# courtois-neuromod/phantom_vlb

Measured on AMD Instinct MI355X. Metric: clips/sec fine-tune VideoLLaMA2-7B+LoRA->2k-voxel head, 1/2/4/8 MI355X, higher is better.
Workload: dtype bf16; 1 GPU; configs[2]: VideoLLaMA2-7B + LoRA r=16 + 2k-voxel head, bf16; clips_per_gpu=3, global_batch=3, seq_len=2048, frames=12, num_target=2048, weights=random-init, comm=none

## Files before the change

### include/vlb.h

```cpp
#ifndef VLB_H
#define VLB_H

#include <stdint.h>

#ifdef __cplusplus
extern "C" {
#endif
#if defined(__GNUC__) || defined(__clang__)
#pragma GCC visibility push(default)
#endif

#define VLB_OK 0
#define VLB_ERR_INVALID (-1)
#define VLB_ERR_LAUNCH (-2)

#define VLB_ABI_VERSION 2

#define VLB_ACT_NONE 0
#define VLB_ACT_QUICK_GELU 1
#define VLB_ACT_GELU 2
#define VLB_ACT_SILU 3
#define VLB_ACT_SWIGLU_PAIR 4
#define VLB_ACT_SWIGLU_BWD 5

// ... 8 lines not shown
                     const void* bias, const void* residual, int ldr, int act, const void* A2, int lda2,
                     const void* W2, int ldw2, int K2, void* ws, int64_t ws_bytes, void* stream);
int vlb_gemm_swiglu_save(const void* A, int lda, const void* W_il, int ldw, void* H, int ldh, void* GU, int ldgu, int M, int N,
                         int K, const void* A2, int lda2, const void* W2_il, int ldw2, int K2, void* ws, int64_t ws_bytes,
                         void* stream);
int64_t vlb_gemm_workspace_bytes(void);
int vlb_gemm_plan(int M, int N, int K, int K2, int with_workspace);

int vlb_gemm_bf16_masked_pair(const void* A, int lda, const void* W, int ldw, void* C, int ldc, int M, int N, int K,
                              const void* A2, int lda2, const void* W2, int ldw2, float drop_p, uint32_t seed,
                              void* stream);

int vlb_gemm_bf16_masked_pair_ws(const void* A, int lda, const void* W, int ldw, void* C, int ldc, int M, int N, int K,
                                 const void* A2, int lda2, const void* W2, int ldw2, float drop_p, uint32_t seed,
                                 void* ws, int64_t ws_bytes, void* stream);

int vlb_gemm_masked_pair_swiglu_bwd(const void* dY, int lddy, const void* Wt, int ldw, const void* gu, int ldgu, void* dgu,
                                    int lddgu, int M, int ff, int K, const void* U, int ldu, const void* At, int ldat,
                                    float drop_p, uint32_t seed, void* ws, int64_t ws_bytes, void* stream);

int vlb_gemm_kernel_choice(int M, int N, int K, int K2);

int vlb_transpose_bf16(const void* in, void* out, int R, int C, void* stream);

int vlb_attention_fwd(const void* q, int ldq, const void* k, int ldk, const void* v, int ldv, void* out, int ldo,
                      float* lse, const uint8_t* key_mask, int B, int S, int Hq, int Hkv, int D, int causal,
                      float scale, const int* cu_rows, void* stream);

int vlb_attention_bwd(const void* q, int ldq, const void* k, int ldk, const void* v, int ldv, const void* out,
                      int ldo, const void* dout, int lddo, const float* lse, const uint8_t* key_mask, void* dq,
                      int lddq, void* dk, int lddk, void* dv, int lddv, float* delta, float* dq_acc, int B, int S,
                      int Hq, int Hkv, int D, int causal, float scale, const int* cu_rows, int total_rows,
                      void* stream);

int vlb_rmsnorm_fwd(const void* x, const void* w, void* y, int rows, int dim, float eps, void* stream);
int vlb_rmsnorm_bwd(const void* x, const void* w, const void* dy, const void* dx_in, void* dx, int rows, int dim,
                    float eps, void* stream);
int vlb_layernorm_fwd(const void* x, const void* w, const void* b, const void* residual, void* y, int rows, int dim,
                      float eps, int act, void* stream);

int vlb_rope_inplace(void* x, int ld, const float* cos_t, const float* sin_t, int rows, int S, int heads, int D,
                     int sign, const int* pos, void* stream);
int vlb_swiglu_fwd(const void* gu, void* out, int rows, int ff, void* stream);
int vlb_swiglu_bwd(const void* gu, const void* dout, void* dgu, int rows, int ff, void* stream);
int vlb_add_bf16(const void* a, const void* b, void* y, int64_t n, void* stream);

int vlb_patchify(const float* vision, void* patches, int N, int H, int W, int P, int Kpad, void* stream);
int vlb_vit_assemble(const void* patch_emb, const void* cls, const void* pos, void* tokens, int N, int G, int D,
                     void* stream);
int vlb_drop_cls(const void* tokens, void* out, int N, int G, int D, void* stream);

int vlb_dwconv3x3(const void* x, const void* w, void* y, int N, int H, int W, int C, void* stream);
int vlb_se_pool(const void* x, void* pooled, int N, int HW, int C, void* stream);
int vlb_se_scale(const void* x, const void* gate, void* y, int N, int HW, int C, void* stream);
int vlb_im2col3d_k2s2p1(const void* x, void* cols, int B, int T, int H, int W, int C, void* stream);

int vlb_splice_embed(const int64_t* ids, const void* embed_w, const void* video_tokens, void* embeds,
                     uint8_t* key_mask, int* err_flag, int B, int L, int Nv, int D, int64_t video_id, int vocab,
                     const int* cu_rows, int* row_pos, void* stream);
int vlb_weight_mask(const int64_t* padvals, const double* vis_w, const double* lang_w, float* wmask, int B, int F,
                    int Lw, int tokens_per_frame, int S, int round_bf16, void* stream);

int vlb_head_partial_rows(int S);
int64_t vlb_head_ws_floats(int B, int S, int E, int V);
int vlb_head_fwd(const void* hidden, const float* wmask, const void* ln1_w, const void* ln1_b, const void* ln2_w,
                 const void* ln2_b, const void* ridge_w, const void* ridge_b, const float* y, const float* keep_scale,
// ... 204 lines not shown
```

### phantom_vlb_amd/_lib.py

```python
from __future__ import annotations

import ctypes
import os
from ctypes import c_char_p, c_double, c_float, c_int, c_int64, c_void_p

import torch

_HERE = os.path.dirname(os.path.abspath(__file__))
LIB_PATH = os.environ.get("VLB_LIB") or os.path.join(_HERE, "libvlb.so")
IS_PRODUCT_LIB = os.path.abspath(LIB_PATH) == os.path.join(_HERE, "libvlb.so")

P, I, F, L, D = c_void_p, c_int, c_float, c_int64, c_double

SIGNATURES = {
    "vlb_abi_version": [],
    "vlb_last_error": [],
    "vlb_gemm_bf16": [P, I, P, I, P, I, I, I, I, P, P, I, I, P, I, P, I, I, P],
    "vlb_gemm_bf16_ws": [P, I, P, I, P, I, I, I, I, P, P, I, I, P, I, P, I, I, P, L, P],
    "vlb_gemm_swiglu_save": [P, I, P, I, P, I, P, I, I, I, I, P, I, P, I, I, P, L, P],
    "vlb_gemm_workspace_bytes": [],
    "vlb_gemm_plan": [I, I, I, I, I],
    "vlb_gemm_kernel_choice": [I, I, I, I],
    "vlb_transpose_bf16": [P, P, I, I, P],
    "vlb_attention_fwd": [P, I, P, I, P, I, P, I, P, P, I, I, I, I, I, I, F, P, P],
    "vlb_attention_bwd": [P, I, P, I, P, I, P, I, P, I, P, P, P, I, P, I, P, I, P, P, I, I, I, I, I, I, F, P, I, P],
    "vlb_rmsnorm_fwd": [P, P, P, I, I, F, P],
    "vlb_rmsnorm_bwd": [P, P, P, P, P, I, I, F, P],
    "vlb_layernorm_fwd": [P, P, P, P, P, I, I, F, I, P],
    "vlb_rope_inplace": [P, I, P, P, I, I, I, I, I, P, P],
    "vlb_swiglu_fwd": [P, P, I, I, P],
    "vlb_swiglu_bwd": [P, P, P, I, I, P],
    "vlb_add_bf16": [P, P, P, L, P],
    "vlb_patchify": [P, P, I, I, I, I, I, P],
    "vlb_vit_assemble": [P, P, P, P, I, I, I, P],
    "vlb_drop_cls": [P, P, I, I, I, P],
    "vlb_dwconv3x3": [P, P, P, I, I, I, I, P],
    "vlb_se_pool": [P, P, I, I, I, P],
    "vlb_se_scale": [P, P, P, I, I, I, P],
    "vlb_im2col3d_k2s2p1": [P, P, I, I, I, I, I, P],
    "vlb_splice_embed": [P, P, P, P, P, P, I, I, I, I, L, I, P, P, P],
    "vlb_weight_mask": [P, P, P, P, I, I, I, I, I, I, P],
    "vlb_head_partial_rows": [I],
    "vlb_head_ws_floats": [I, I, I, I],
    "vlb_head_fwd": [P] * 19 + [I, I, I, I, F, F, P, P],
    "vlb_head_bwd": [P] * 24 + [I, I, I, I, F, F, F, F, P, I, P],
    "vlb_feature_cache_store": [P] * 5 + [I, I, I, P],
    "vlb_head_fwd_cached": [P] * 19 + [I, I, I, I, F, F, P],
    "vlb_head_bwd_cached": [P] * 20 + [I, I, I, F, F, F, F, P],
    "vlb_head_loss_fwd": [P] * 6 + [I, I, I, I, I, F, P],
    "vlb_head_bwd_loss": [P] * 24 + [I, I, I, I, F, F, F, F, P, I, P, I, P],
    "vlb_head_bwd_cached_loss": [P] * 20 + [I, I, I, F, F, F, F, P, I, P],
    "vlb_head_grouped_ws_floats": [I, I, I, I],
    "vlb_head_fwd_grouped": [P] * 22 + [I, I, I, I, I, F, F, I, P],
    "vlb_head_bwd_grouped": [P] * 22 + [I, I, I, I, F, F, F, F, I, P],
    "vlb_head_pool": [P] * 6 + [I, I, I, F, P, P],
    "vlb_feature_cache_gather": [P] * 5 + [I, I, I, P],
    "vlb_head_mix_fwd": [P] * 4 + [I, I, I, P],
    "vlb_head_mix_ws_floats": [I, I, I],
# ... 118 lines not shown
```

### phantom_vlb_amd/backbone.py

```python
from __future__ import annotations

import math

import torch

from . import ops
from .geometry import Geometry, VIDEO_TOKEN_ID, decoder_linears

BF16 = torch.bfloat16
V_PRE = "model.vision_tower.vision_tower.vision_model"
M_PRE = "model.mm_projector"


def _bf(t, dev):
    return t.detach().to(device=dev, dtype=BF16).contiguous()


class Weights:

    def __init__(self, g: Geometry, sd: dict, device, keep_transposed: bool = False, gate_up_interleaved: bool | None = None):
        self.g = g
        self.dev = device
        d = device
        w = sd[f"{V_PRE}.embeddings.patch_embedding.weight"].reshape(g.vit_dim, -1)
        wp = torch.zeros(g.vit_dim, g.patch_k_padded, dtype=w.dtype, device=w.device)
        wp[:, :g.patch_k] = w
        self.patch_w = _bf(wp, d)
        self.cls = _bf(sd[f"{V_PRE}.embeddings.class_embedding"], d)
        self.pos = _bf(sd[f"{V_PRE}.embeddings.position_embedding.weight"], d)
        self.pre_ln = (_bf(sd[f"{V_PRE}.pre_layrnorm.weight"], d), _bf(sd[f"{V_PRE}.pre_layrnorm.bias"], d))
        self.vit = []
        for i in range(g.vit_layers_run):
            p = f"{V_PRE}.encoder.layers.{i}"
            a = f"{p}.self_attn"
            self.vit.append(dict(
                ln1=(_bf(sd[f"{p}.layer_norm1.weight"], d), _bf(sd[f"{p}.layer_norm1.bias"], d)),
                ln2=(_bf(sd[f"{p}.layer_norm2.weight"], d), _bf(sd[f"{p}.layer_norm2.bias"], d)),
                wqkv=_bf(torch.cat([sd[f"{a}.q_proj.weight"], sd[f"{a}.k_proj.weight"], sd[f"{a}.v_proj.weight"]], 0), d),
                bqkv=_bf(torch.cat([sd[f"{a}.q_proj.bias"], sd[f"{a}.k_proj.bias"], sd[f"{a}.v_proj.bias"]], 0), d),
                wo=_bf(sd[f"{a}.out_proj.weight"], d), bo=_bf(sd[f"{a}.out_proj.bias"], d),
                w1=_bf(sd[f"{p}.mlp.fc1.weight"], d), b1=_bf(sd[f"{p}.mlp.fc1.bias"], d),
                w2=_bf(sd[f"{p}.mlp.fc2.weight"], d), b2=_bf(sd[f"{p}.mlp.fc2.bias"], d)))
        def stage(prefix):
            blocks = []
# ... 158 lines not shown
        y = ops.layernorm(y, *blk["bn2"], g.proj_eps, act=ops.ACT_SILU)
        s = ops.se_pool(y, N, H * H, C)
        s = ops.gemm(s, blk["se1"], bias=blk["se1b"], act=ops.ACT_SILU)
        s = ops.gemm(s, blk["se2"], bias=blk["se2b"])
        y = ops.se_scale(y, s, N, H * H, C, out=y)
        y = ops.gemm(y, blk["conv3"])
        sc = x
        if "ds" in blk:
            sc = ops.layernorm(ops.gemm(x, blk["ds"]), *blk["dsbn"], g.proj_eps)
        return ops.layernorm(y, *blk["bn3"], g.proj_eps, residual=sc, act=ops.ACT_SILU)

    def connector(self, feats, B):
        g, w = self.g, self.w
        x = feats
        for blk in w.s1:
            x = self._bottleneck(x, blk, B * g.num_frames, g.grid)
        cols = ops.im2col3d(x, B, g.num_frames, g.grid, g.grid, g.dim)
        x = ops.gemm(cols, w.sampler_w, bias=w.sampler_b, act=ops.ACT_SILU)
        for blk in w.s2:
            x = self._bottleneck(x, blk, B * g.ds_frames, g.ds_grid)
        x = ops.gemm(x, w.ro0[0], bias=w.ro0[1], act=ops.ACT_GELU)
        return ops.gemm(x, w.ro2[0], bias=w.ro2[1])

    def attention(self, qkv, key_mask, B, layout=None, need_lse=False):
        g, w = self.g, self.w
        qd, kd = g.q_dim, g.kv_dim
        ops.rope_(qkv, w.rope_cos, w.rope_sin, B, g.max_len, g.heads + g.kv_heads, g.head_dim,
                  pos=None if layout is None else layout.pos)
        return ops.attention_fwd(qkv[:, :qd], qkv[:, qd:qd + kd], qkv[:, qd + kd:], B, g.max_len, g.heads, g.kv_heads,
                                 g.head_dim, True, g.head_dim ** -0.5, key_mask=key_mask, need_lse=need_lse, layout=layout)

    def attention_bwd(self, qkv, a, d_a, lse, key_mask, B, layout, delta):
        g, w = self.g, self.w
        dqkv = ops.attention_bwd(qkv, g.q_dim, g.kv_dim, a, d_a, lse, key_mask, B, g.max_len, g.heads, g.kv_heads,
                                 g.head_dim, True, g.head_dim ** -0.5, layout=layout, delta=delta)
        ops.rope_(dqkv, w.rope_cos, w.rope_sin, B, g.max_len, g.heads + g.kv_heads, g.head_dim, sign=-1,
                  pos=None if layout is None else layout.pos)
        return dqkv

    def decoder_layer(self, x, lw, key_mask, B, S, save=None, layout=None):
        g = self.g
        assert S == g.max_len, "the decoder runs at the geometry's sequence length (rope tables, attention)"
        h = ops.rmsnorm(x, lw["in_norm"], g.rms_eps)
        qkv = ops.gemm(h, lw["wqkv"])
        a = self.attention(qkv, key_mask, B, layout)
        x = ops.gemm(a, lw["wo"], residual=x)
        h = ops.rmsnorm(x, lw["post_norm"], g.rms_eps)
        if lw.get("wgu_il") is not None:
            h = ops.gemm(h, lw["wgu_il"], act=ops.ACT_SWIGLU_PAIR)
        else:
            h = ops.swiglu(ops.gemm(h, lw["wgu"]))
        return ops.gemm(h, lw["wdown"], residual=x)

    def named_modules(self):
        from .litmodule import _LinearInfo
        g = self.g
        for i in range(g.vit_layers):
            p = f"{V_PRE}.encoder.layers.{i}"
            for n in ("q_proj", "k_proj", "v_proj", "out_proj"):
                yield f"{p}.self_attn.{n}", _LinearInfo(g.vit_dim, g.vit_dim)
            yield f"{p}.mlp.fc1", _LinearInfo(g.vit_ff, g.vit_dim)
            yield f"{p}.mlp.fc2", _LinearInfo(g.vit_dim, g.vit_ff)
        for n in ("readout.0", "readout.2"):
            yield f"{M_PRE}.{n}", _LinearInfo(g.dim, g.dim)
        for i in range(g.layers):
            p = f"model.layers.{i}"
# ... 155 lines not shown
```

### phantom_vlb_amd/csrc/attention.hip

```cpp
#include "common.hpp"

namespace {

constexpr int KV = 64;
constexpr int QW = 32;
constexpr int NW = 4;
constexpr int QB = QW * NW;
constexpr float NEG = -1e30f;

typedef short s16x4 __attribute__((ext_vector_type(4)));

__device__ __forceinline__ s16x4 tr_read_asm(const char* lds_ptr) {
  s16x4 v;
  const unsigned a = (unsigned)(uintptr_t)(const char __attribute__((address_space(3)))*)lds_ptr;
  asm volatile("ds_read_b64_tr_b16 %0, %1" : "=v"(v) : "v"(a));
  return v;
}
__device__ __forceinline__ void lds_wait_all() {
  asm volatile("s_waitcnt lgkmcnt(0)" ::: "memory");
  __builtin_amdgcn_sched_barrier(0);
}
__device__ __forceinline__ bf16x8 join8(s16x4 lo, s16x4 hi) {
  typedef short s16x8 __attribute__((ext_vector_type(8)));
  return __builtin_bit_cast(bf16x8, (s16x8)__builtin_shufflevector(lo, hi, 0, 1, 2, 3, 4, 5, 6, 7));
// ... 421 lines not shown
        for (int dt = 0; dt < 4; ++dt)
          dvt[dt] = __builtin_amdgcn_mfma_f32_32x32x16_bf16(join8(ra[dt][0], ra[dt][1]), pb[s], dvt[dt], 0, 0, 0);
#pragma unroll
        for (int dt = 0; dt < 4; ++dt)
#pragma unroll
          for (int e = 0; e < 2; ++e) ra[dt][e] = tr_read_asm(qt + qt_rd[dt][e] + 16 * s * ROWB);
        lds_wait_all();
#pragma unroll
        for (int dt = 0; dt < 4; ++dt)
          dkt[dt] = __builtin_amdgcn_mfma_f32_32x32x16_bf16(join8(ra[dt][0], ra[dt][1]), dsb[s], dkt[dt], 0, 0, 0);
      }
    }
    asm volatile("s_waitcnt vmcnt(0)" ::: "memory");
    asm volatile("s_waitcnt lgkmcnt(0)" ::: "memory");
    __builtin_amdgcn_s_barrier();
  }

  if (key < Sb) {
    bf16* dkp = gsz == 1 ? p.dk + (row0 + key) * p.lddk + hkv * D : part + ((row0 + key) * p.Hq + hq) * (2 * D);
    bf16* dvp = gsz == 1 ? p.dv + (row0 + key) * p.lddv + hkv * D : dkp + D;
#pragma unroll
    for (int dt = 0; dt < 4; ++dt)
#pragma unroll
      for (int g = 0; g < 4; ++g) {
        bf16x4 a, c;
#pragma unroll
        for (int e = 0; e < 4; ++e) { a[e] = (bf16)dkt[dt][4 * g + e]; c[e] = (bf16)dvt[dt][4 * g + e]; }
        *reinterpret_cast<bf16x4*>(dkp + 32 * dt + 8 * g + 4 * h) = a;
        *reinterpret_cast<bf16x4*>(dvp + 32 * dt + 8 * g + 4 * h) = c;
      }
  }
}

__global__ __launch_bounds__(256) void attn_dkdv_reduce_kernel(const bf16* __restrict__ part, bf16* __restrict__ dk, int lddk,
                                                               bf16* __restrict__ dv, int lddv, int Hq, int Hkv, int64_t total) {
  const int64_t i = blockIdx.x * (int64_t)blockDim.x + threadIdx.x;
  if (i >= total) return;
  const int c = i & 15, which = (i >> 4) & 1;
  const int hkv = (int)((i >> 5) % Hkv);
  const int64_t row = (i >> 5) / Hkv;
  const int gsz = Hq / Hkv;
  float acc[8] = {0.f, 0.f, 0.f, 0.f, 0.f, 0.f, 0.f, 0.f};
  const bf16* src = part + (row * Hq + (int64_t)hkv * gsz) * 256 + which * 128 + c * 8;
  for (int j = 0; j < gsz; ++j) {
    const bf16x8 v = *reinterpret_cast<const bf16x8*>(src + (int64_t)j * 256);
#pragma unroll
    for (int e = 0; e < 8; ++e) acc[e] += (float)v[e];
  }
  bf16x8 o;
#pragma unroll
  for (int e = 0; e < 8; ++e) o[e] = (bf16)acc[e];
  bf16* dst = which ? dv + row * lddv : dk + row * lddk;
  *reinterpret_cast<bf16x8*>(dst + hkv * 128 + c * 8) = o;
}

struct AttnDqArgs {
  const bf16* q; const bf16* k; const bf16* v; const bf16* dout;
  const float* lse; const float* delta; const uint8_t* mask; const int* cu;
  bf16* dq;
  int ldq, ldk, ldv, lddo, lddq;
  int B, S, Hq, Hkv;
  float scale;
};

template <bool CAUSAL>
__global__ __launch_bounds__(256, 2) void attn_bwd_dq_kernel(AttnDqArgs p) {
  constexpr int D = 128, ROWB = 256, TILE = KV * ROWB, KS = 8, DT = 4;
  extern __shared__ __attribute__((aligned(16))) char smem[];

  const int tid = threadIdx.x, lane = tid & 63;
  const int wave = __builtin_amdgcn_readfirstlane(tid >> 6);
  const int nqb = (p.S + QB - 1) / QB;
  const int per_qb = p.Hq * p.B, slot = blockIdx.x / per_qb;
  const int qb = CAUSAL ? (nqb - 1 - slot) : slot;
  const int hq = xcd_head((blockIdx.x % per_qb) % p.Hq, p.Hq), b = (blockIdx.x % per_qb) / p.Hq;
  const int hkv = hq / (p.Hq / p.Hkv);
  const int Sb = p.cu ? p.cu[b + 1] - p.cu[b] : p.S;
  const int64_t row0 = p.cu ? p.cu[b] : (int64_t)b * p.S;
  if (qb * QB >= Sb) return;
  const int q0 = qb * QB + wave * QW;
  const int ql = lane & 31, h = lane >> 5;
  const int qrow = q0 + ql;
  const int qr = min(qrow, Sb - 1);

  bf16x8 qf[KS], dof[KS];
  {
    const bf16* qp = p.q + (row0 + qr) * p.ldq + hq * D + 8 * h;
    const bf16* dp = p.dout + (row0 + qr) * p.lddo + hq * D + 8 * h;
#pragma unroll
    for (int ks = 0; ks < KS; ++ks) {
      qf[ks] = *reinterpret_cast<const bf16x8*>(qp + 16 * ks);
      dof[ks] = *reinterpret_cast<const bf16x8*>(dp + 16 * ks);
    }
  }
  const float lse_q = p.lse[((int64_t)b * p.Hq + hq) * p.S + qr];
  const float delta_q = p.delta[((int64_t)b * p.Hq + hq) * p.S + qr];
  const float c2 = p.scale * 1.44269504088896341f;
  const float lse2 = (lse_q > -1e37f) ? lse_q * 1.44269504088896341f : 1e37f;

  f32x16 dqt[DT];
#pragma unroll
  for (int i = 0; i < DT; ++i)
#pragma unroll
    for (int r = 0; r < 16; ++r) dqt[i][r] = 0.f;

  const int q_hi = min(qb * QB + QB, Sb) - 1;
  const int ntiles = CAUSAL ? (q_hi / KV + 1) : (Sb + KV - 1) / KV;
  const bf16* kbase = p.k + row0 * p.ldk + hkv * D;
  const bf16* vbase = p.v + row0 * p.ldv + hkv * D;

  const int sr = lane >> 4, sp = lane & 15;
  auto stage = [&](int buf, int t) {
    char* kb = smem + buf * 2 * TILE; char* vb = kb + TILE;
#pragma unroll
    for (int i = 0; i < 4; ++i) {
      const int r = (4 * i + wave) * 4 + sr;
      const int key = min(t * KV + r, Sb - 1);
      glds16(kbase + (int64_t)key * p.ldk + (sp ^ sw2(r)) * 8, kb + (4 * i + wave) * 1024);
      glds16(vbase + (int64_t)key * p.ldv + (sp ^ sw2(r)) * 8, vb + (4 * i + wave) * 1024);
    }
  };
  stage(0, 0);
  asm volatile("s_waitcnt vmcnt(0)" ::: "memory");
  __syncthreads();

  const int g1 = (lane >> 4) & 1, li = lane & 15, tq = li >> 2, tp = li & 3;
  int row_rd[KS];
#pragma unroll
  for (int ks = 0; ks < KS; ++ks) row_rd[ks] = ql * ROWB + (((2 * ks + h) ^ sw2(ql)) << 4);
  int tr_rd[DT][2];
#pragma unroll
  for (int dt = 0; dt < DT; ++dt)
#pragma unroll
    for (int e = 0; e < 2; ++e) {
      const int r = 4 * h + tq + 8 * e;
      tr_rd[dt][e] = r * ROWB + (((4 * dt + 2 * g1 + (tp >> 1)) ^ sw2(r)) << 4) + (tp & 1) * 8;
    }

  for (int t = 0; t < ntiles; ++t) {
    const int cur = t & 1;
    if (t + 1 < ntiles) stage(cur ^ 1, t + 1);
    const char* kb = smem + cur * 2 * TILE; const char* vb = kb + TILE;
    const int key0 = t * KV;
    const bool active = !CAUSAL || (key0 <= q0 + QW - 1);
    if (active) {
      f32x16 st[2], dp[2];
#pragma unroll
      for (int s = 0; s < 2; ++s)
#pragma unroll
        for (int r = 0; r < 16; ++r) { st[s][r] = 0.f; dp[s][r] = 0.f; }
#pragma unroll
      for (int ks = 0; ks < KS; ++ks) {
#pragma unroll
        for (int s = 0; s < 2; ++s) {
// ... 28 lines not shown
        asm volatile("" ::: "memory");
      }
#pragma unroll
      for (int s = 0; s < 2; ++s)
#pragma unroll
        for (int r = 0; r < 16; ++r) {
          const float pv = __builtin_amdgcn_exp2f(st[s][r] * c2 - lse2);
          st[s][r] = pv * (dp[s][r] - delta_q) * p.scale;
        }
#pragma unroll
      for (int s = 0; s < 2; ++s)
#pragma unroll
        for (int s2 = 0; s2 < 2; ++s2) {
          bf16x8 df;
#pragma unroll
          for (int j = 0; j < 8; ++j) df[j] = (bf16)st[s][8 * s2 + j];
          const int roff = (32 * s + 16 * s2) * ROWB;
#pragma unroll
          for (int dt = 0; dt < DT; ++dt) {
            const s16x4 lo = __builtin_amdgcn_ds_read_tr16_b64_v4i16(
                (s16x4 __attribute__((address_space(3)))*)(kb + tr_rd[dt][0] + roff));
            const s16x4 hi = __builtin_amdgcn_ds_read_tr16_b64_v4i16(
                (s16x4 __attribute__((address_space(3)))*)(kb + tr_rd[dt][1] + roff));
            dqt[dt] = __builtin_amdgcn_mfma_f32_32x32x16_bf16(join8(lo, hi), df, dqt[dt], 0, 0, 0);
          }
        }
    }
    asm volatile("s_waitcnt vmcnt(0)" ::: "memory");
    __syncthreads();
  }

  if (qrow < Sb) {
    bf16* op = p.dq + (row0 + qrow) * p.lddq + hq * D;
#pragma unroll
    for (int dt = 0; dt < DT; ++dt)
#pragma unroll
      for (int g = 0; g < 4; ++g) {
        bf16x4 o;
#pragma unroll
        for (int e = 0; e < 4; ++e) o[e] = (bf16)dqt[dt][4 * g + e];
        *reinterpret_cast<bf16x4*>(op + 32 * dt + 8 * g + 4 * h) = o;
      }
  }
}

}

extern "C" int vlb_attention_bwd(const void* q, int ldq, const void* k, int ldk, const void* v, int ldv, const void* out,
                                 int ldo, const void* dout, int lddo, const float* lse, const uint8_t* key_mask, void* dq,
                                 int lddq, void* dk, int lddk, void* dv, int lddv, float* delta, float* dq_acc, int B,
                                 int S, int Hq, int Hkv, int D, int causal, float scale, const int* cu_rows, int total_rows,
                                 void* stream) {
  VLB_REQUIRE(q && k && v && out && dout && lse && dq && dk && dv && delta, "attention_bwd: null operand");
  VLB_REQUIRE(dq_acc || Hq == Hkv, "attention_bwd: the [rows, Hq, D] fp32-sized workspace is required");
  VLB_REQUIRE(D == 128, "attention_bwd: head dim %d unsupported (only 128: the decoder)", D);
  VLB_REQUIRE(B > 0 && S > 0 && Hq > 0 && Hkv > 0 && Hq % Hkv == 0, "attention_bwd: bad shape");
  VLB_REQUIRE(ldq % 8 == 0 && ldk % 8 == 0 && ldv % 8 == 0 && ldo % 8 == 0 && lddo % 8 == 0 && lddq % 8 == 0 &&
                  lddk % 4 == 0 && lddv % 4 == 0, "attention_bwd: strides must keep vector alignment");
  VLB_REQUIRE(((((uintptr_t)q | (uintptr_t)k | (uintptr_t)v | (uintptr_t)out | (uintptr_t)dout) % 16) == 0) &&
                  ((uintptr_t)dq % 8 == 0), "attention_bwd: misaligned pointer");
  hipStream_t st = as_stream(stream);
  const int64_t rows = cu_rows ? (int64_t)total_rows : (int64_t)B * S;
  VLB_REQUIRE(rows > 0 && rows <= (int64_t)B * S, "attention_bwd: total_rows=%d out of range", total_rows);
  const int64_t th = rows * Hq;
  hipLaunchKernelGGL(attn_delta_kernel, dim3((unsigned)((th + 15) / 16)), dim3(256), 0, st, (const bf16*)out, ldo,
                     (const bf16*)dout, lddo, delta, S, Hq, B, cu_rows, th);
  VLB_LAUNCH_CHECK();
  AttnBwdArgs a{(const bf16*)q, (const bf16*)k, (const bf16*)v, (const bf16*)dout, lse, delta, key_mask, cu_rows,
                (bf16*)dk, (bf16*)dv, dq_acc, ldq, ldk, ldv, lddo, lddk, lddv, B, S, Hq, Hkv, scale, g_attn_ablate};
  dim3 grid((S + BK_KEYS - 1) / BK_KEYS, Hkv, B);
  {
    const int gsz = Hq / Hkv;
    VLB_REQUIRE(gsz == 1 || dq_acc, "attention_bwd: the workspace (fp32 [rows, Hq, D]) is required for grouped-query heads");
    VLB_REQUIRE(lddk % 8 == 0 && lddv % 8 == 0 && (((uintptr_t)dk | (uintptr_t)dv) % 16) == 0, "attention_bwd: dk/dv rows must be 16-byte aligned");
    constexpr int LDS_KV = BK_KEYS * 256 + 4 * BQ * 256 + 512;
    static const hipError_t k1 = hipFuncSetAttribute(reinterpret_cast<const void*>(&attn_bwd_dkdv_kernel<true>), hipFuncAttributeMaxDynamicSharedMemorySize, LDS_KV);
    static const hipError_t k2 = hipFuncSetAttribute(reinterpret_cast<const void*>(&attn_bwd_dkdv_kernel<false>), hipFuncAttributeMaxDynamicSharedMemorySize, LDS_KV);
    if (k1 != hipSuccess || k2 != hipSuccess) { vlb_set_error("attention_bwd: LDS reservation failed (dk/dv)"); return VLB_ERR_LAUNCH; }
    bf16* part = reinterpret_cast<bf16*>(dq_acc);
    dim3 gridh(grid.x * Hq * B);
    if (causal) hipLaunchKernelGGL(attn_bwd_dkdv_kernel<true>, gridh, dim3(256), LDS_KV, st, a, part);
    else hipLaunchKernelGGL(attn_bwd_dkdv_kernel<false>, gridh, dim3(256), LDS_KV, st, a, part);
    VLB_LAUNCH_CHECK();
    if (gsz > 1) {
      const int64_t tot = rows * Hkv * 32;
      hipLaunchKernelGGL(attn_dkdv_reduce_kernel, dim3((unsigned)((tot + 255) / 256)), dim3(256), 0, st, part, (bf16*)dk, lddk,
                         (bf16*)dv, lddv, Hq, Hkv, tot);
      VLB_LAUNCH_CHECK();
    }
  }
  AttnDqArgs d{(const bf16*)q, (const bf16*)k, (const bf16*)v, (const bf16*)dout, lse, delta, key_mask, cu_rows,
               (bf16*)dq, ldq, ldk, ldv, lddo, lddq, B, S, Hq, Hkv, scale};
  constexpr int LDS_DQ = 2 * 2 * KV * 256;
  static const hipError_t q1 = hipFuncSetAttribute(reinterpret_cast<const void*>(&attn_bwd_dq_kernel<true>), hipFuncAttributeMaxDynamicSharedMemorySize, LDS_DQ);
  static const hipError_t q2 = hipFuncSetAttribute(reinterpret_cast<const void*>(&attn_bwd_dq_kernel<false>), hipFuncAttributeMaxDynamicSharedMemorySize, LDS_DQ);
  if (q1 != hipSuccess || q2 != hipSuccess) { vlb_set_error("attention_bwd: LDS reservation failed (dq)"); return VLB_ERR_LAUNCH; }
  dim3 gq(((S + QB - 1) / QB) * Hq * B);
  if (causal) hipLaunchKernelGGL(attn_bwd_dq_kernel<true>, gq, dim3(256), LDS_DQ, st, d);
  else hipLaunchKernelGGL(attn_bwd_dq_kernel<false>, gq, dim3(256), LDS_DQ, st, d);
  VLB_LAUNCH_CHECK();
  return VLB_OK;
}

#ifdef VLB_TOOLS
extern "C" void vlb_attn_set_ablation(int bits) { g_attn_ablate = bits & 3; }
#endif
```

### phantom_vlb_amd/ops.py

```python
from __future__ import annotations

import torch

from ._lib import check, lib

ACT_NONE, ACT_QUICK_GELU, ACT_GELU, ACT_SILU, ACT_SWIGLU_PAIR = 0, 1, 2, 3, 4
BF16 = torch.bfloat16


def _stream():
    return torch.cuda.current_stream().cuda_stream


def _p(t):
    return None if t is None else t.data_ptr()


def _dev(t):
    if not t.is_cuda:
        raise RuntimeError("phantom_vlb_amd ops need GPU tensors (no CPU fallback)")
    return t


class _GemmProbe:
# ... 240 lines not shown

_ATTN_WS = [None]


def _attn_workspace(n_floats, device):
    ws = _ATTN_WS[0]
    if ws is None or ws.numel() < n_floats or ws.device != device:
        ws = _ATTN_WS[0] = torch.empty(n_floats, dtype=torch.float32, device=device)
    return ws


def attention_bwd(qkv, qd, kd, out, dout, lse, key_mask, B, S, Hq, Hkv, D, causal, scale, layout=None, delta=None,
                  dq_acc=None):
    cu, rows = None, B * S
    if layout is not None and layout.packed:
        B, S, cu, rows = layout.B, layout.smax, layout.cu, layout.rows
    assert qkv.shape[0] == rows and dout.shape[0] == rows
    if delta is None:
        delta = torch.empty(B, Hq, S, dtype=torch.float32, device=qkv.device)
    if dq_acc is None and Hq != Hkv:
        dq_acc = _attn_workspace(rows * qd, qkv.device)
    assert delta.numel() >= B * Hq * S and (dq_acc is None or dq_acc.numel() >= rows * qd)
    dqkv = torch.empty_like(qkv)
    check(lib.vlb_attention_bwd(qkv.data_ptr(), qkv.stride(0), qkv[:, qd:].data_ptr(), qkv.stride(0),
                                qkv[:, qd + kd:].data_ptr(), qkv.stride(0), out.data_ptr(), out.stride(0),
                                dout.data_ptr(), dout.stride(0), lse.data_ptr(), _p(key_mask),
                                dqkv.data_ptr(), dqkv.stride(0), dqkv[:, qd:].data_ptr(), dqkv.stride(0),
                                dqkv[:, qd + kd:].data_ptr(), dqkv.stride(0), delta.data_ptr(), _p(dq_acc),
                                B, S, Hq, Hkv, D, 1 if causal else 0, float(scale), _p(cu), rows, _stream()),
          "vlb_attention_bwd")
    return dqkv


def rmsnorm(x, w, eps, out=None):
    rows, dim = x.shape
    if out is None:
        out = torch.empty_like(x)
    check(lib.vlb_rmsnorm_fwd(_dev(x).data_ptr(), w.data_ptr(), out.data_ptr(), rows, dim, eps, _stream()), "vlb_rmsnorm_fwd")
    return out


def rmsnorm_bwd(x, w, dy, eps, dx_in=None, out=None):
    rows, dim = x.shape
    if out is None:
        out = torch.empty_like(x)
    check(lib.vlb_rmsnorm_bwd(_dev(x).data_ptr(), w.data_ptr(), dy.data_ptr(), _p(dx_in), out.data_ptr(), rows, dim, eps,
                              _stream()), "vlb_rmsnorm_bwd")
    return out


def layernorm(x, w, b, eps, residual=None, act=ACT_NONE, out=None):
    rows, dim = x.shape
    if out is None:
        out = torch.empty_like(x)
    check(lib.vlb_layernorm_fwd(_dev(x).data_ptr(), w.data_ptr(), b.data_ptr(), _p(residual), out.data_ptr(), rows, dim,
                                eps, act, _stream()), "vlb_layernorm_fwd")
    return out


def rope_(x, cos, sin, B, S, heads, D, sign=1, pos=None):
    rows = B * S if pos is None else pos.shape[0]
    assert x.shape[0] == rows and cos.shape[0] >= S
    check(lib.vlb_rope_inplace(_dev(x).data_ptr(), x.stride(0), cos.data_ptr(), sin.data_ptr(), rows, S, heads, D, sign,
                               _p(pos), _stream()), "vlb_rope_inplace")
    return x

# ... 278 lines not shown
```

Before: 15.19 clips/s.

## Fold RoPE undo and delta computation into GQA attention backward kernels

Adds a RoPE-folded attention backward path. The dq kernel now computes delta = rowsum(out·dout) itself and writes it out for the dk/dv kernel, so dq is launched before dk/dv and the separate delta kernel goes away. The inverse-RoPE rotation is applied in the dq epilogue and in the dk reduce kernel, which removes the standalone rope_ pass over dqkv. This saves two launches and a full read/write of dqkv per layer. In exchange the dq kernel does extra loads of out and the cos/sin tables, and the two kernels now have a new ordering dependency.

Result: no change. 15.26 clips/s, median of 6 (+0.4%).

```diff
diff --git a/include/vlb.h b/include/vlb.h
--- a/include/vlb.h
+++ b/include/vlb.h
@@ -64,6 +64,11 @@
                       int lddq, void* dk, int lddk, void* dv, int lddv, float* delta, float* dq_acc, int B, int S,
                       int Hq, int Hkv, int D, int causal, float scale, const int* cu_rows, int total_rows,
                       void* stream);
+int vlb_attention_bwd_rope(const void* q, int ldq, const void* k, int ldk, const void* v, int ldv, const void* out,
+                           int ldo, const void* dout, int lddo, const float* lse, const uint8_t* key_mask, void* dq,
+                           int lddq, void* dk, int lddk, void* dv, int lddv, float* delta, float* dq_acc, int B, int S,
+                           int Hq, int Hkv, int D, int causal, float scale, const int* cu_rows, int total_rows,
+                           const float* cos_t, const float* sin_t, const int* pos, void* stream);
 
 int vlb_rmsnorm_fwd(const void* x, const void* w, void* y, int rows, int dim, float eps, void* stream);
 int vlb_rmsnorm_bwd(const void* x, const void* w, const void* dy, const void* dx_in, void* dx, int rows, int dim,
diff --git a/phantom_vlb_amd/_lib.py b/phantom_vlb_amd/_lib.py
--- a/phantom_vlb_amd/_lib.py
+++ b/phantom_vlb_amd/_lib.py
@@ -24,6 +24,7 @@
     "vlb_transpose_bf16": [P, P, I, I, P],
     "vlb_attention_fwd": [P, I, P, I, P, I, P, I, P, P, I, I, I, I, I, I, F, P, P],
     "vlb_attention_bwd": [P, I, P, I, P, I, P, I, P, I, P, P, P, I, P, I, P, I, P, P, I, I, I, I, I, I, F, P, I, P],
+    "vlb_attention_bwd_rope": [P, I, P, I, P, I, P, I, P, I, P, P, P, I, P, I, P, I, P, P, I, I, I, I, I, I, F, P, I, P, P, P, P],
     "vlb_rmsnorm_fwd": [P, P, P, I, I, F, P],
     "vlb_rmsnorm_bwd": [P, P, P, P, P, I, I, F, P],
     "vlb_layernorm_fwd": [P, P, P, P, P, I, I, F, I, P],
diff --git a/phantom_vlb_amd/backbone.py b/phantom_vlb_amd/backbone.py
--- a/phantom_vlb_amd/backbone.py
+++ b/phantom_vlb_amd/backbone.py
@@ -10,6 +10,7 @@
 BF16 = torch.bfloat16
 V_PRE = "model.vision_tower.vision_tower.vision_model"
 M_PRE = "model.mm_projector"
+FOLD_ATTN_BWD_ROPE = True
 
 
 def _bf(t, dev):
@@ -234,6 +235,10 @@
 
     def attention_bwd(self, qkv, a, d_a, lse, key_mask, B, layout, delta):
         g, w = self.g, self.w
+        if FOLD_ATTN_BWD_ROPE:
+            return ops.attention_bwd_rope(qkv, g.q_dim, g.kv_dim, a, d_a, lse, key_mask, B, g.max_len, g.heads, g.kv_heads,
+                                          g.head_dim, True, g.head_dim ** -0.5, w.rope_cos, w.rope_sin, layout=layout,
+                                          delta=delta)
         dqkv = ops.attention_bwd(qkv, g.q_dim, g.kv_dim, a, d_a, lse, key_mask, B, g.max_len, g.heads, g.kv_heads,
                                  g.head_dim, True, g.head_dim ** -0.5, layout=layout, delta=delta)
         ops.rope_(dqkv, w.rope_cos, w.rope_sin, B, g.max_len, g.heads + g.kv_heads, g.head_dim, sign=-1,
diff --git a/phantom_vlb_amd/csrc/attention.hip b/phantom_vlb_amd/csrc/attention.hip
--- a/phantom_vlb_amd/csrc/attention.hip
+++ b/phantom_vlb_amd/csrc/attention.hip
@@ -477,8 +477,29 @@
   }
 }
 
+__device__ __forceinline__ float dot8_in_order(bf16x8 a, bf16x8 b) {
+#pragma clang fp contract(off)
+  float s = 0.f;
+#pragma unroll
+  for (int i = 0; i < 8; ++i) s += (float)a[i] * (float)b[i];
+  return s;
+}
+__device__ __forceinline__ float rope_undo_lo(float a, float b, float co, float sn) {
+#pragma clang fp contract(off)
+  const float si = -sn;
+  return __builtin_fmaf(a, co, -(b * si));
+}
+__device__ __forceinline__ float rope_undo_hi(float a, float b, float co, float sn) {
+#pragma clang fp contract(off)
+  const float si = -sn;
+  return __builtin_fmaf(b, co, a * si);
+}
+
+template <bool ROPE>
 __global__ __launch_bounds__(256) void attn_dkdv_reduce_kernel(const bf16* __restrict__ part, bf16* __restrict__ dk, int lddk,
-                                                               bf16* __restrict__ dv, int lddv, int Hq, int Hkv, int64_t total) {
+                                                               bf16* __restrict__ dv, int lddv, int Hq, int Hkv, int64_t total,
+                                                               const float* __restrict__ cs, const float* __restrict__ sn,
+                                                               const int* __restrict__ pos, int S) {
   const int64_t i = blockIdx.x * (int64_t)blockDim.x + threadIdx.x;
   if (i >= total) return;
   const int c = i & 15, which = (i >> 4) & 1;
@@ -486,6 +507,13 @@
   const int64_t row = (i >> 5) / Hkv;
   const int gsz = Hq / Hkv;
   float acc[8] = {0.f, 0.f, 0.f, 0.f, 0.f, 0.f, 0.f, 0.f};
+  f32x4 c0, c1, s0, s1;
+  if (ROPE && which == 0) {
+    const int s = pos ? pos[row] : (int)(row % S);
+    const int64_t t = (int64_t)s * 64 + (c & 7) * 8;
+    c0 = *reinterpret_cast<const f32x4*>(cs + t); c1 = *reinterpret_cast<const f32x4*>(cs + t + 4);
+    s0 = *reinterpret_cast<const f32x4*>(sn + t); s1 = *reinterpret_cast<const f32x4*>(sn + t + 4);
+  }
   const bf16* src = part + (row * Hq + (int64_t)hkv * gsz) * 256 + which * 128 + c * 8;
   for (int j = 0; j < gsz; ++j) {
     const bf16x8 v = *reinterpret_cast<const bf16x8*>(src + (int64_t)j * 256);
@@ -495,6 +523,19 @@
   bf16x8 o;
 #pragma unroll
   for (int e = 0; e < 8; ++e) o[e] = (bf16)acc[e];
+  if (ROPE && which == 0) {
+    const u32x4 mine = __builtin_bit_cast(u32x4, o);
+    u32x4 theirs;
+#pragma unroll
+    for (int j = 0; j < 4; ++j) theirs[j] = __shfl_xor(mine[j], 8, 64);
+    const bf16x8 other = __builtin_bit_cast(bf16x8, theirs);
+#pragma unroll
+    for (int e = 0; e < 8; ++e) {
+      const float co = e < 4 ? c0[e & 3] : c1[e & 3], si = e < 4 ? s0[e & 3] : s1[e & 3];
+      const float a = (float)(c < 8 ? o[e] : other[e]), b = (float)(c < 8 ? other[e] : o[e]);
+      o[e] = (bf16)(c < 8 ? rope_undo_lo(a, b, co, si) : rope_undo_hi(a, b, co, si));
+    }
+  }
   bf16* dst = which ? dv + row * lddv : dk + row * lddk;
   *reinterpret_cast<bf16x8*>(dst + hkv * 128 + c * 8) = o;
 }
@@ -506,9 +547,11 @@
   int ldq, ldk, ldv, lddo, lddq;
   int B, S, Hq, Hkv;
   float scale;
+  const bf16* out; float* delta_w; const float* cs; const float* sn; const int* pos;
+  int ldo;
 };
 
-template <bool CAUSAL>
+template <bool CAUSAL, bool FOLD = false>
 __global__ __launch_bounds__(256, 2) void attn_bwd_dq_kernel(AttnDqArgs p) {
   constexpr int D = 128, ROWB = 256, TILE = KV * ROWB, KS = 8, DT = 4;
   extern __shared__ __attribute__((aligned(16))) char smem[];
@@ -539,7 +582,10 @@
     }
   }
   const float lse_q = p.lse[((int64_t)b * p.Hq + hq) * p.S + qr];
-  const float delta_q = p.delta[((int64_t)b * p.Hq + hq) * p.S + qr];
+  float delta_q = 0.f;
+  int rope_s = 0;
+  if constexpr (FOLD) rope_s = p.pos ? p.pos[row0 + qr] : (int)((row0 + qr) % p.S);
+  else delta_q = p.delta[((int64_t)b * p.Hq + hq) * p.S + qr];
   const float c2 = p.scale * 1.44269504088896341f;
   const float lse2 = (lse_q > -1e37f) ? lse_q * 1.44269504088896341f : 1e37f;
 
@@ -565,6 +611,15 @@
       glds16(vbase + (int64_t)key * p.ldv + (sp ^ sw2(r)) * 8, vb + (4 * i + wave) * 1024);
     }
   };
+  if constexpr (FOLD) {
+    const bf16* op = p.out + (row0 + qr) * p.ldo + hq * D + 8 * h;
+    float t[KS];
+#pragma unroll
+    for (int ks = 0; ks < KS; ++ks) t[ks] = dot8_in_order(*reinterpret_cast<const bf16x8*>(op + 16 * ks), dof[ks]);
+    const float w = ((t[0] + t[4]) + (t[2] + t[6])) + ((t[1] + t[5]) + (t[3] + t[7]));
+    delta_q = w + __shfl_xor(w, 32, 64);
+    if (h == 0 && qrow < Sb) p.delta_w[((int64_t)b * p.Hq + hq) * p.S + qrow] = delta_q;
+  }
   stage(0, 0);
   asm volatile("s_waitcnt vmcnt(0)" ::: "memory");
   __syncthreads();
@@ -659,25 +714,52 @@
 
   if (qrow < Sb) {
     bf16* op = p.dq + (row0 + qrow) * p.lddq + hq * D;
-#pragma unroll
-    for (int dt = 0; dt < DT; ++dt)
-#pragma unroll
-      for (int g = 0; g < 4; ++g) {
-        bf16x4 o;
-#pragma unroll
-        for (int e = 0; e < 4; ++e) o[e] = (bf16)dqt[dt][4 * g + e];
-        *reinterpret_cast<bf16x4*>(op + 32 * dt + 8 * g + 4 * h) = o;
-      }
-  }
-}
-
-}
-
-extern "C" int vlb_attention_bwd(const void* q, int ldq, const void* k, int ldk, const void* v, int ldv, const void* out,
-                                 int ldo, const void* dout, int lddo, const float* lse, const uint8_t* key_mask, void* dq,
-                                 int lddq, void* dk, int lddk, void* dv, int lddv, float* delta, float* dq_acc, int B,
-                                 int S, int Hq, int Hkv, int D, int causal, float scale, const int* cu_rows, int total_rows,
-                                 void* stream) {
+    if constexpr (FOLD) {
+      const float* cp = p.cs + (int64_t)rope_s * (D / 2) + 4 * h;
+      const float* sp2 = p.sn + (int64_t)rope_s * (D / 2) + 4 * h;
+      f32x4 co[2][4], si[2][4];
+#pragma unroll
+      for (int dt = 0; dt < 2; ++dt)
+#pragma unroll
+        for (int g = 0; g < 4; ++g) {
+          co[dt][g] = *reinterpret_cast<const f32x4*>(cp + 32 * dt + 8 * g);
+          si[dt][g] = *reinterpret_cast<const f32x4*>(sp2 + 32 * dt + 8 * g);
+        }
+#pragma unroll
+      for (int dt = 0; dt < 2; ++dt)
+#pragma unroll
+        for (int g = 0; g < 4; ++g) {
+          bf16x4 lo, hi;
+#pragma unroll
+          for (int e = 0; e < 4; ++e) {
+            const float a = (float)(bf16)dqt[dt][4 * g + e], b2 = (float)(bf16)dqt[dt + 2][4 * g + e];
+            lo[e] = (bf16)rope_undo_lo(a, b2, co[dt][g][e], si[dt][g][e]);
+            hi[e] = (bf16)rope_undo_hi(a, b2, co[dt][g][e], si[dt][g][e]);
+          }
+          *reinterpret_cast<bf16x4*>(op + 32 * dt + 8 * g + 4 * h) = lo;
+          *reinterpret_cast<bf16x4*>(op + 64 + 32 * dt + 8 * g + 4 * h) = hi;
+        }
+    } else {
+#pragma unroll
+      for (int dt = 0; dt < DT; ++dt)
+#pragma unroll
+        for (int g = 0; g < 4; ++g) {
+          bf16x4 o;
+#pragma unroll
+          for (int e = 0; e < 4; ++e) o[e] = (bf16)dqt[dt][4 * g + e];
+          *reinterpret_cast<bf16x4*>(op + 32 * dt + 8 * g + 4 * h) = o;
+        }
+    }
+  }
+}
+
+}
+
+static int attention_bwd_run(const void* q, int ldq, const void* k, int ldk, const void* v, int ldv, const void* out, int ldo,
+                             const void* dout, int lddo, const float* lse, const uint8_t* key_mask, void* dq, int lddq,
+                             void* dk, int lddk, void* dv, int lddv, float* delta, float* dq_acc, int B, int S, int Hq,
+                             int Hkv, int D, int causal, float scale, const int* cu_rows, int total_rows, bool fold,
+                             const float* cos_t, const float* sin_t, const int* pos, void* stream) {
   VLB_REQUIRE(q && k && v && out && dout && lse && dq && dk && dv && delta, "attention_bwd: null operand");
   VLB_REQUIRE(dq_acc || Hq == Hkv, "attention_bwd: the [rows, Hq, D] fp32-sized workspace is required");
   VLB_REQUIRE(D == 128, "attention_bwd: head dim %d unsupported (only 128: the decoder)", D);
@@ -686,47 +768,90 @@
                   lddk % 4 == 0 && lddv % 4 == 0, "attention_bwd: strides must keep vector alignment");
   VLB_REQUIRE(((((uintptr_t)q | (uintptr_t)k | (uintptr_t)v | (uintptr_t)out | (uintptr_t)dout) % 16) == 0) &&
                   ((uintptr_t)dq % 8 == 0), "attention_bwd: misaligned pointer");
+  if (fold) {
+    VLB_REQUIRE(Hq != Hkv, "attention_bwd_rope: needs grouped-query heads (Hq=%d, Hkv=%d)", Hq, Hkv);
+    VLB_REQUIRE(cos_t && sin_t && (((uintptr_t)cos_t | (uintptr_t)sin_t) % 16) == 0, "attention_bwd_rope: cos/sin tables missing or misaligned");
+    VLB_REQUIRE(pos || !cu_rows, "attention_bwd_rope: packed rows need their positions");
+  }
   hipStream_t st = as_stream(stream);
   const int64_t rows = cu_rows ? (int64_t)total_rows : (int64_t)B * S;
   VLB_REQUIRE(rows > 0 && rows <= (int64_t)B * S, "attention_bwd: total_rows=%d out of range", total_rows);
-  const int64_t th = rows * Hq;
-  hipLaunchKernelGGL(attn_delta_kernel, dim3((unsigned)((th + 15) / 16)), dim3(256), 0, st, (const bf16*)out, ldo,
-                     (const bf16*)dout, lddo, delta, S, Hq, B, cu_rows, th);
-  VLB_LAUNCH_CHECK();
+  const int gsz = Hq / Hkv;
+  VLB_REQUIRE(gsz == 1 || dq_acc, "attention_bwd: the workspace (fp32 [rows, Hq, D]) is required for grouped-query heads");
+  VLB_REQUIRE(lddk % 8 == 0 && lddv % 8 == 0 && (((uintptr_t)dk | (uintptr_t)dv) % 16) == 0, "attention_bwd: dk/dv rows must be 16-byte aligned");
+
+  auto launch_dq = [&]() -> int {
+    AttnDqArgs d{(const bf16*)q, (const bf16*)k, (const bf16*)v, (const bf16*)dout, lse, delta, key_mask, cu_rows,
+                 (bf16*)dq, ldq, ldk, ldv, lddo, lddq, B, S, Hq, Hkv, scale,
+                 (const bf16*)out, delta, cos_t, sin_t, pos, ldo};
+    constexpr int LDS_DQ = 2 * 2 * KV * 256;
+    static const hipError_t q1 = hipFuncSetAttribute(reinterpret_cast<const void*>(&attn_bwd_dq_kernel<true>), hipFuncAttributeMaxDynamicSharedMemorySize, LDS_DQ);
+    static const hipError_t q2 = hipFuncSetAttribute(reinterpret_cast<const void*>(&attn_bwd_dq_kernel<false>), hipFuncAttributeMaxDynamicSharedMemorySize, LDS_DQ);
+    static const hipError_t q3 = hipFuncSetAttribute(reinterpret_cast<const void*>(&attn_bwd_dq_kernel<true, true>), hipFuncAttributeMaxDynamicSharedMemorySize, LDS_DQ);
+    static const hipError_t q4 = hipFuncSetAttribute(reinterpret_cast<const void*>(&attn_bwd_dq_kernel<false, true>), hipFuncAttributeMaxDynamicSharedMemorySize, LDS_DQ);
+    if (q1 != hipSuccess || q2 != hipSuccess || q3 != hipSuccess || q4 != hipSuccess) { vlb_set_error("attention_bwd: LDS reservation failed (dq)"); return VLB_ERR_LAUNCH; }
+    dim3 gq(((S + QB - 1) / QB) * Hq * B);
+    if (fold) {
+      if (causal) hipLaunchKernelGGL((attn_bwd_dq_kernel<true, true>), gq, dim3(256), LDS_DQ, st, d);
+      else hipLaunchKernelGGL((attn_bwd_dq_kernel<false, true>), gq, dim3(256), LDS_DQ, st, d);
+    } else {
+      if (causal) hipLaunchKernelGGL(attn_bwd_dq_kernel<true>, gq, dim3(256), LDS_DQ, st, d);
+      else hipLaunchKernelGGL(attn_bwd_dq_kernel<false>, gq, dim3(256), LDS_DQ, st, d);
+    }
+    VLB_LAUNCH_CHECK();
+    return VLB_OK;
+  };
+
+  if (fold) {
+    if (const int rc = launch_dq()) return rc;
+  } else {
+    const int64_t th = rows * Hq;
+    hipLaunchKernelGGL(attn_delta_kernel, dim3((unsigned)((th + 15) / 16)), dim3(256), 0, st, (const bf16*)out, ldo,
+                       (const bf16*)dout, lddo, delta, S, Hq, B, cu_rows, th);
+    VLB_LAUNCH_CHECK();
+  }
   AttnBwdArgs a{(const bf16*)q, (const bf16*)k, (const bf16*)v, (const bf16*)dout, lse, delta, key_mask, cu_rows,
                 (bf16*)dk, (bf16*)dv, dq_acc, ldq, ldk, ldv, lddo, lddk, lddv, B, S, Hq, Hkv, scale, g_attn_ablate};
-  dim3 grid((S + BK_KEYS - 1) / BK_KEYS, Hkv, B);
   {
-    const int gsz = Hq / Hkv;
-    VLB_REQUIRE(gsz == 1 || dq_acc, "attention_bwd: the workspace (fp32 [rows, Hq, D]) is required for grouped-query heads");
-    VLB_REQUIRE(lddk % 8 == 0 && lddv % 8 == 0 && (((uintptr_t)dk | (uintptr_t)dv) % 16) == 0, "attention_bwd: dk/dv rows must be 16-byte aligned");
     constexpr int LDS_KV = BK_KEYS * 256 + 4 * BQ * 256 + 512;
     static const hipError_t k1 = hipFuncSetAttribute(reinterpret_cast<const void*>(&attn_bwd_dkdv_kernel<true>), hipFuncAttributeMaxDynamicSharedMemorySize, LDS_KV);
     static const hipError_t k2 = hipFuncSetAttribute(reinterpret_cast<const void*>(&attn_bwd_dkdv_kernel<false>), hipFuncAttributeMaxDynamicSharedMemorySize, LDS_KV);
     if (k1 != hipSuccess || k2 != hipSuccess) { vlb_set_error("attention_bwd: LDS reservation failed (dk/dv)"); return VLB_ERR_LAUNCH; }
     bf16* part = reinterpret_cast<bf16*>(dq_acc);
-    dim3 gridh(grid.x * Hq * B);
+    dim3 gridh(((S + BK_KEYS - 1) / BK_KEYS) * Hq * B);
     if (causal) hipLaunchKernelGGL(attn_bwd_dkdv_kernel<true>, gridh, dim3(256), LDS_KV, st, a, part);
     else hipLaunchKernelGGL(attn_bwd_dkdv_kernel<false>, gridh, dim3(256), LDS_KV, st, a, part);
     VLB_LAUNCH_CHECK();
     if (gsz > 1) {
       const int64_t tot = rows * Hkv * 32;
-      hipLaunchKernelGGL(attn_dkdv_reduce_kernel, dim3((unsigned)((tot + 255) / 256)), dim3(256), 0, st, part, (bf16*)dk, lddk,
-                         (bf16*)dv, lddv, Hq, Hkv, tot);
+      const dim3 gr((unsigned)((tot + 255) / 256));
+      if (fold) hipLaunchKernelGGL(attn_dkdv_reduce_kernel<true>, gr, dim3(256), 0, st, part, (bf16*)dk, lddk, (bf16*)dv, lddv,
+                                   Hq, Hkv, tot, cos_t, sin_t, pos, S);
+      else hipLaunchKernelGGL(attn_dkdv_reduce_kernel<false>, gr, dim3(256), 0, st, part, (bf16*)dk, lddk, (bf16*)dv, lddv,
+                              Hq, Hkv, tot, (const float*)nullptr, (const float*)nullptr, (const int*)nullptr, S);
       VLB_LAUNCH_CHECK();
     }
   }
-  AttnDqArgs d{(const bf16*)q, (const bf16*)k, (const bf16*)v, (const bf16*)dout, lse, delta, key_mask, cu_rows,
-               (bf16*)dq, ldq, ldk, ldv, lddo, lddq, B, S, Hq, Hkv, scale};
-  constexpr int LDS_DQ = 2 * 2 * KV * 256;
-  static const hipError_t q1 = hipFuncSetAttribute(reinterpret_cast<const void*>(&attn_bwd_dq_kernel<true>), hipFuncAttributeMaxDynamicSharedMemorySize, LDS_DQ);
-  static const hipError_t q2 = hipFuncSetAttribute(reinterpret_cast<const void*>(&attn_bwd_dq_kernel<false>), hipFuncAttributeMaxDynamicSharedMemorySize, LDS_DQ);
-  if (q1 != hipSuccess || q2 != hipSuccess) { vlb_set_error("attention_bwd: LDS reservation failed (dq)"); return VLB_ERR_LAUNCH; }
-  dim3 gq(((S + QB - 1) / QB) * Hq * B);
-  if (causal) hipLaunchKernelGGL(attn_bwd_dq_kernel<true>, gq, dim3(256), LDS_DQ, st, d);
-  else hipLaunchKernelGGL(attn_bwd_dq_kernel<false>, gq, dim3(256), LDS_DQ, st, d);
-  VLB_LAUNCH_CHECK();
-  return VLB_OK;
+  return fold ? VLB_OK : launch_dq();
+}
+
+extern "C" int vlb_attention_bwd(const void* q, int ldq, const void* k, int ldk, const void* v, int ldv, const void* out,
+                                 int ldo, const void* dout, int lddo, const float* lse, const uint8_t* key_mask, void* dq,
+                                 int lddq, void* dk, int lddk, void* dv, int lddv, float* delta, float* dq_acc, int B,
+                                 int S, int Hq, int Hkv, int D, int causal, float scale, const int* cu_rows, int total_rows,
+                                 void* stream) {
+  return attention_bwd_run(q, ldq, k, ldk, v, ldv, out, ldo, dout, lddo, lse, key_mask, dq, lddq, dk, lddk, dv, lddv, delta,
+                           dq_acc, B, S, Hq, Hkv, D, causal, scale, cu_rows, total_rows, false, nullptr, nullptr, nullptr,
+                           stream);
+}
+
+extern "C" int vlb_attention_bwd_rope(const void* q, int ldq, const void* k, int ldk, const void* v, int ldv, const void* out,
+                                      int ldo, const void* dout, int lddo, const float* lse, const uint8_t* key_mask,
+                                      void* dq, int lddq, void* dk, int lddk, void* dv, int lddv, float* delta, float* dq_acc,
+                                      int B, int S, int Hq, int Hkv, int D, int causal, float scale, const int* cu_rows,
+                                      int total_rows, const float* cos_t, const float* sin_t, const int* pos, void* stream) {
+  return attention_bwd_run(q, ldq, k, ldk, v, ldv, out, ldo, dout, lddo, lse, key_mask, dq, lddq, dk, lddk, dv, lddv, delta,
+                           dq_acc, B, S, Hq, Hkv, D, causal, scale, cu_rows, total_rows, true, cos_t, sin_t, pos, stream);
 }
 
 #ifdef VLB_TOOLS
diff --git a/phantom_vlb_amd/ops.py b/phantom_vlb_amd/ops.py
--- a/phantom_vlb_amd/ops.py
+++ b/phantom_vlb_amd/ops.py
@@ -296,6 +296,36 @@
     return dqkv
 
 
+def attention_bwd_rope(qkv, qd, kd, out, dout, lse, key_mask, B, S, Hq, Hkv, D, causal, scale, cos, sin, layout=None,
+                       delta=None, dq_acc=None, pos=None):
+    if pos is None and layout is not None:
+        pos = layout.pos
+    packed = layout is not None and layout.packed
+    if Hq == Hkv or D != 128 or (packed and pos is None):
+        dqkv = attention_bwd(qkv, qd, kd, out, dout, lse, key_mask, B, S, Hq, Hkv, D, causal, scale, layout=layout,
+                             delta=delta, dq_acc=dq_acc)
+        return rope_(dqkv, cos, sin, B, S, Hq + Hkv, D, sign=-1, pos=pos)
+    cu, rows = None, B * S
+    if packed:
+        B, S, cu, rows = layout.B, layout.smax, layout.cu, layout.rows
+    assert qkv.shape[0] == rows and dout.shape[0] == rows and cos.shape[0] >= S and (pos is None or pos.shape[0] == rows)
+    if delta is None:
+        delta = torch.empty(B, Hq, S, dtype=torch.float32, device=qkv.device)
+    if dq_acc is None:
+        dq_acc = _attn_workspace(rows * qd, qkv.device)
+    assert delta.numel() >= B * Hq * S and dq_acc.numel() >= rows * qd
+    dqkv = torch.empty_like(qkv)
+    check(lib.vlb_attention_bwd_rope(qkv.data_ptr(), qkv.stride(0), qkv[:, qd:].data_ptr(), qkv.stride(0),
+                                     qkv[:, qd + kd:].data_ptr(), qkv.stride(0), out.data_ptr(), out.stride(0),
+                                     dout.data_ptr(), dout.stride(0), lse.data_ptr(), _p(key_mask),
+                                     dqkv.data_ptr(), dqkv.stride(0), dqkv[:, qd:].data_ptr(), dqkv.stride(0),
+                                     dqkv[:, qd + kd:].data_ptr(), dqkv.stride(0), delta.data_ptr(), _p(dq_acc),
+                                     B, S, Hq, Hkv, D, 1 if causal else 0, float(scale), _p(cu), rows,
+                                     cos.data_ptr(), sin.data_ptr(), _p(pos), _stream()),
+          "vlb_attention_bwd_rope")
+    return dqkv
+
+
 def rmsnorm(x, w, eps, out=None):
     rows, dim = x.shape
     if out is None:
```
